# RaduAlexandru/permuto_sdf

Measured on AMD Instinct MI355X. Metric: ray-samples/sec (encode+MLP+composite), higher is better.
Workload: dtype f32 (MLP products on 2 fp16 operand pieces per fp32 value, fp32 accumulation; the 3-piece / 24-bit figure is value_fp32_equivalent_24bit)

## Files before the change

permuto_sdf_amd/csrc/encode.hip:

```cpp
#include <cstdlib>
#include <cstdio>
#include "encode_device.h"
#include <vector>
#include <mutex>
#include <cstring>

namespace {

template <int P, int F, bool PLAIN = false>
__global__ void __launch_bounds__(PSDF_BLOCK)
    encode_fwd_kernel(int64_t N, int L, uint32_t capacity, EncConv conv, const float* __restrict__ positions,
                      const float* __restrict__ lattice, const float* __restrict__ scale_factor,
                      const float* __restrict__ shifts, const float* __restrict__ window, float points_scaling,
                      int pad_points, const unsigned char* __restrict__ skip, float* __restrict__ sliced,
                      unsigned char* __restrict__ touched, int touch_shift, int blocks_per_level) {
  const int level = blockIdx.y;
  const int64_t ntiles = (N + PSDF_BLOCK - 1) / PSDF_BLOCK;
  for (int64_t tile = blockIdx.x; tile < ntiles; tile += gridDim.x) {
  const int64_t n = tile * PSDF_BLOCK + threadIdx.x;
  if (n >= N) continue;
  if (!PLAIN && skip && skip[n]) continue;
  float pos[P];
  load_pos<P>(positions, n, pos);
  if (level >= L) {
// ... 83 lines not shown
  constexpr int ROW_SHR = 0x110, ROW_SHL = 0x100;
  const int k = (int)key;
  const int kprev = __builtin_amdgcn_update_dpp(0, k, ROW_SHR | 1, 0xf, 0xf, true);
  const float joined = (kprev == k) ? 1.0f : 0.0f;
  float j = joined;
#define PSDF_SCAN_STEP(D)                                                                                        \
  {                                                                                                              \
    _Pragma("unroll") for (int i = 0; i < F; i++) v[i] = __builtin_fmaf(                                         \
        __int_as_float(__builtin_amdgcn_update_dpp(0, __float_as_int(v[i]), ROW_SHR | D, 0xf, 0xf, true)), j, v[i]); \
    j = j * __int_as_float(__builtin_amdgcn_update_dpp(0, __float_as_int(j), ROW_SHR | D, 0xf, 0xf, true));      \
  }
  PSDF_SCAN_STEP(1)
  PSDF_SCAN_STEP(2)
  PSDF_SCAN_STEP(4)
  PSDF_SCAN_STEP(8)
#undef PSDF_SCAN_STEP
  const int next_joined = __builtin_amdgcn_update_dpp(0, __float_as_int(joined), ROW_SHL | 1, 0xf, 0xf, true);
  return key != Q_NONE && next_joined == 0;
}

template <int F, int TOTAL = 8192>
struct ScatterCache {
  static constexpr int SC_SLOTS = TOTAL / F;
  uint32_t* tags;
  float* sums;
  int* stats;
  __device__ __forceinline__ void init(float* lds) {
    tags = reinterpret_cast<uint32_t*>(lds);
    sums = lds + SC_SLOTS;
    stats = reinterpret_cast<int*>(lds + SC_SLOTS + SC_SLOTS * F);
    for (int i = threadIdx.x; i < SC_SLOTS; i += blockDim.x) tags[i] = SC_EMPTY;
    for (int i = threadIdx.x; i < SC_SLOTS * F; i += blockDim.x) sums[i] = 0.f;
    if (threadIdx.x == 0) {
      stats[0] = 0;
      stats[1] = 0;
      stats[2] = 1;
    }
    __syncthreads();
  }
  __device__ __forceinline__ int add(uint32_t row, const float* v, int& hot) {
    const uint32_t slot = (row ^ (row >> 12)) & (SC_SLOTS - 1);
    uint32_t old = tags[slot];
    if (old == SC_EMPTY) old = atomicCAS(&tags[slot], SC_EMPTY, row);
    if (old == SC_EMPTY || old == row) {
      static_assert(F % 2 == 0, "pairs");
#pragma unroll
      for (int f = 0; f < F; f += 2) lds_add_pair(&sums[slot * F + f], v[f], v[f + 1], hot);
      return old == row ? 2 : 1;
    }
    return 0;
  }
  __device__ __forceinline__ void flush(float* __restrict__ table_grad) {
    __syncthreads();
    for (int i = threadIdx.x; i < SC_SLOTS; i += blockDim.x) {
      const uint32_t row = tags[i];
      if (row != SC_EMPTY) {
#pragma unroll
        for (int f = 0; f < F; f++) {
          const float v = sums[i * F + f];
          if (v != 0.f) atomicAdd(table_grad + (int64_t)row * F + f, v);
        }
      }
    }
  }
  static constexpr size_t bytes() { return (size_t)(SC_SLOTS + SC_SLOTS * F + 4) * 4; }
};

template <typename SC>
__device__ __forceinline__ bool cache_vote(SC& sc, int hits, int tries) {
  hits = (int)psdf::wave_sum((float)hits);
  tries = (int)psdf::wave_sum((float)tries);
  if (psdf::lane_id() == 0) {
    atomicAdd(&sc.stats[0], hits);
    atomicAdd(&sc.stats[1], tries);
  }
  __syncthreads();
  return sc.stats[0] * 8 >= sc.stats[1];
}

struct Queues {
  uint16_t* rows;
  float* vals;
  int* tails;
  int cap, np, shift;
};
constexpr int Q_MAX_PARTS = 64;
constexpr int Q_LDS_INTS = 4 * Q_MAX_PARTS + 4;

struct LevelQueues {
  char* rows;
  char* vals;
  uint32_t mask;
};
template <int F>
__device__ __forceinline__ LevelQueues level_queues(const Queues& Q, int level) {
  const int64_t e = (int64_t)level * Q.np * Q.cap;
  return LevelQueues{reinterpret_cast<char*>(Q.rows + e), reinterpret_cast<char*>(Q.vals + e * F), (1u << Q.shift) - 1u};
}
template <int F>
__device__ __forceinline__ void queue_store(const LevelQueues& LQ, uint32_t o, uint32_t row, const float* v) {
  *reinterpret_cast<uint16_t*>(LQ.rows + (o * 2u)) = (uint16_t)(row & LQ.mask);
  if (F == 2) {
    *reinterpret_cast<float2*>(LQ.vals + (o * 8u)) = make_float2(v[0], v[F - 1]);
  } else {
#pragma unroll
    for (int f = 0; f < F; f++) *reinterpret_cast<float*>(LQ.vals + (o * (uint32_t)(F * 4) + (uint32_t)(f * 4))) = v[f];
  }
}

template <int NC, int F>
__device__ __forceinline__ void queue_push(const Queues& Q, int level, int* q_cnt, int* q_base,
                                           const uint32_t (&crow)[NC], const float (&cval)[NC][F],
                                           float* __restrict__ table_grad) {
  int* q_aux = q_base + Q_MAX_PARTS;
  const LevelQueues LQ = level_queues<F>(Q, level);
  if (threadIdx.x < Q.np) q_cnt[threadIdx.x] = 0;
  __syncthreads();
  int slot[NC];
#pragma unroll
  for (int r = 0; r < NC; r++)
    if (crow[r] != Q_NONE) slot[r] = atomicAdd(&q_cnt[crow[r] >> Q.shift], 1);
  __syncthreads();
  if (threadIdx.x < Q.np) {
    const int c = q_cnt[threadIdx.x];
    const int base = c ? atomicAdd(&Q.tails[level * Q.np + threadIdx.x], c) : 0;
    q_base[threadIdx.x] = base;
    q_aux[threadIdx.x] = (int)threadIdx.x * Q.cap + base;
  }
  __syncthreads();
#pragma unroll
  for (int r = 0; r < NC; r++) {
    if (crow[r] == Q_NONE) continue;
    const int part = crow[r] >> Q.shift;
    const int idx = q_base[part] + slot[r];
    if (idx < Q.cap) {
      queue_store<F>(LQ, (uint32_t)(q_aux[part] + slot[r]), crow[r], cval[r]);
    } else {
#pragma unroll
      for (int f = 0; f < F; f++) atomicAdd(table_grad + (int64_t)crow[r] * F + f, cval[r][f]);
    }
  }
}

template <int NC>
__device__ __forceinline__ void queue_push_staged(const Queues& Q, int level, int* q_cnt, int* q_base, int* q_off, int* q_gd,
                                                  float* stage, const uint32_t (&crow)[NC],
                                                  const float (&cval)[NC][2], float* __restrict__ table_grad) {
  uint32_t* st_row = reinterpret_cast<uint32_t*>(stage);
  float2* st_val = reinterpret_cast<float2*>(stage + NC * PSDF_BLOCK);
  const LevelQueues LQ = level_queues<2>(Q, level);
  if (threadIdx.x < Q.np) q_cnt[threadIdx.x] = 0;
  __syncthreads();
  int slot[NC];
#pragma unroll
  for (int r = 0; r < NC; r++)
    if (crow[r] != Q_NONE) slot[r] = atomicAdd(&q_cnt[crow[r] >> Q.shift], 1);
  __syncthreads();
  if (threadIdx.x < 64) {
    const int lane = threadIdx.x;
    const int c = lane < Q.np ? q_cnt[lane] : 0;
    const int incl = psdf::wave_incl_scan_add_i(c);
    if (lane < Q.np) {
      const int base = c ? atomicAdd(&Q.tails[level * Q.np + lane], c) : 0;
      const int off = incl - c;
      q_off[lane] = off;
      q_base[lane] = base - off;
      q_gd[lane] = lane * Q.cap + base - off;
      if (lane == Q.np - 1) q_off[Q.np] = incl;
// ... 348 lines not shown
#pragma unroll
  for (int li = 0; li < POS_LPB; li++) {
    const int level = blockIdx.y * POS_LPB + li;
    if (level >= Lt) break;
    float g[F];
#pragma unroll
    for (int f = 0; f < F; f++)
      g[f] = (level < L || (level - L) * F + f < P || pad_points) ? grad_sliced[((int64_t)level * F + f) * N + n] : 0.f;
    if (level >= L) {
      const int e = level - L;
#pragma unroll
      for (int f = 0; f < F; f++) {
        const int d = e * F + f;
#pragma unroll
        for (int i = 0; i < P; i++)
          if (i == d) gp[i] = gp[i] + g[f] * points_scaling;
      }
      continue;
    }
    float sfl[P], shl[P];
#pragma unroll
    for (int i = 0; i < P; i++) {
      sfl[i] = scale_factor[level * P + i];
      shl[i] = shifts[level * P + i];
    }
    const float w = window[level];
    if (w == 0.f) continue;
    const int64_t tbase = (int64_t)level * capacity * F;
    Simplex<P> s;
    compute_simplex<P>(pos, shl, sfl, s, conv.tie_later);
    float dbary[P + 2];
#pragma unroll
    for (int k = 0; k <= P + 1; k++) dbary[k] = 0.f;
    uint32_t rows[P + 1];
    vertex_rows<P>(s, capacity, rows, conv.hash_c);
#pragma unroll
    for (int r = 0; r <= P; r++) {
      const uint32_t row = rows[r];
#pragma unroll
      for (int f = 0; f < F; f++) dbary[r] = dbary[r] + lattice[tbase + (int64_t)row * F + f] * w * g[f];
    }
    dbary[P + 1] = dbary[P + 1] + dbary[0];
    float dE[P + 1];
    const float invp = 1.0f / (P + 1);
#pragma unroll
    for (int i = 0; i <= P; i++) {
      float a = 0.f, b = 0.f;
#pragma unroll
      for (int k = 0; k <= P + 1; k++) {
        if (k == P - s.rank[i]) a = dbary[k];
        if (k == P + 1 - s.rank[i]) b = dbary[k];
      }
      dE[i] = (a - b) * invp;
    }
#pragma unroll
    for (int i = 0; i < P; i++) {
      float acc = 0.f;
#pragma unroll
      for (int j = 0; j <= i; j++) acc = acc + dE[j];
      acc = acc - dE[i + 1] * (float)(i + 1);
      gp[i] = gp[i] + acc * sfl[i];
    }
  }
  if (PARTIAL) {
#pragma unroll
    for (int i = 0; i < P; i++) grad_positions[((int64_t)blockIdx.y * N + n) * P + i] = gp[i];
  } else {
#pragma unroll
    for (int i = 0; i < P; i++) atomicAdd(grad_positions + n * P + i, gp[i]);
  }
}

__global__ void __launch_bounds__(PSDF_BLOCK)
    encode_bwd_pos_reduce_kernel(int64_t NP, int P, int groups, const float* __restrict__ partial,
                                 const unsigned char* __restrict__ skip, float* __restrict__ grad_positions) {
  const int64_t e = (int64_t)blockIdx.x * PSDF_BLOCK + threadIdx.x;
  if (e >= NP) return;
  if (skip && skip[e / P]) return;
  float s = partial[e];
  for (int g = 1; g < groups; g++) s = s + partial[(int64_t)g * NP + e];
  grad_positions[e] = grad_positions[e] + s;
}

template <int F>
__global__ void __launch_bounds__(1024)
    encode_bwd_reduce_kernel(uint32_t capacity, Queues Q, float* __restrict__ grad_lattice) {
  extern __shared__ __align__(16) float tab[];
  const int part = blockIdx.x, level = blockIdx.y;
  int n = Q.tails[level * Q.np + part];
  if (n == 0) return;
  if (n > Q.cap) n = Q.cap;
  const int rpp = 1 << Q.shift;
  for (int i = threadIdx.x; i < rpp * F; i += blockDim.x) tab[i] = 0.f;
  __syncthreads();
  const int64_t qb = ((int64_t)level * Q.np + part) * Q.cap;
  const uint16_t* __restrict__ rows = Q.rows + qb;
  const float* __restrict__ vals = Q.vals + qb * F;
#if !defined(PSDF_ENC_REDUCE_U)
#define PSDF_ENC_REDUCE_U 8
#endif
  constexpr int U = PSDF_ENC_REDUCE_U;
  int hot = 0;
  for (int base = 0; base < n; base += U * (int)blockDim.x) {
    int row[U];
    float v[U][F];
#pragma unroll
    for (int u = 0; u < U; u++) {
      const int i = base + u * (int)blockDim.x + (int)threadIdx.x;
      row[u] = (i < n) ? (int)rows[i] : -1;
      if (F == 2) {
        const float2 t = (i < n) ? *reinterpret_cast<const float2*>(vals + (int64_t)i * 2) : make_float2(0.f, 0.f);
        v[u][0] = t.x;
        v[u][F - 1] = t.y;
      } else {
#pragma unroll
        for (int f = 0; f < F; f++) v[u][f] = (i < n) ? vals[(int64_t)i * F + f] : 0.f;
      }
    }
#pragma unroll
    for (int u = 0; u < U; u++)
      if (row[u] >= 0) {
#pragma unroll
        for (int f = 0; f < F; f += 2) lds_add_pair(&tab[row[u] * F + f], v[u][f], v[u][f + 1], hot);
      }
  }
  __syncthreads();
  const int64_t row0 = (int64_t)part << Q.shift;
  int64_t nrows = (int64_t)capacity - row0;
  if (nrows > rpp) nrows = rpp;
  float* __restrict__ out = grad_lattice + ((int64_t)level * capacity + row0) * F;
  for (int64_t i = threadIdx.x; i < nrows * F; i += blockDim.x) {
    const float v = tab[i];
    if (v != 0.f) out[i] = out[i] + v;
  }
}

template <int P, int F, bool LATTICE>
__global__ void __launch_bounds__(PSDF_BLOCK)
    encode_dbl_bwd_kernel(int64_t N, int L, uint32_t capacity, EncConv conv, const float* __restrict__ positions,
                          const float* __restrict__ lattice, const float* __restrict__ scale_factor,
                          const float* __restrict__ shifts, const float* __restrict__ window, float points_scaling,
                          int pad_points, const float* __restrict__ dd_positions, const float* __restrict__ grad_sliced,
                          float* __restrict__ grad_lattice, float* __restrict__ grad_grad_sliced) {
  extern __shared__ __align__(16) float lds[];
  const int level = blockIdx.y;
  const int64_t ntiles = (N + PSDF_BLOCK - 1) / PSDF_BLOCK;
  if (level >= L) {
    const int e = level - L;
    for (int64_t tile = blockIdx.x; tile < ntiles; tile += gridDim.x) {
      const int64_t n = tile * PSDF_BLOCK + threadIdx.x;
      if (n >= N) continue;
      float u[P];
      load_pos<P>(dd_positions, n, u);
#pragma unroll
      for (int f = 0; f < F; f++) {
        const int d = e * F + f;
        float v = 0.f;
#pragma unroll
        for (int i = 0; i < P; i++)
          if (i == d) v = u[i] * points_scaling;
        if (d < P || pad_points) grad_grad_sliced[((int64_t)level * F + f) * N + n] = v;
      }
    }
    return;
  }
  const float w = window[level];
  if (w == 0.f) {
    for (int64_t tile = blockIdx.x; tile < ntiles; tile += gridDim.x) {
      const int64_t n = tile * PSDF_BLOCK + threadIdx.x;
      if (n >= N) continue;
#pragma unroll
      for (int f = 0; f < F; f++) grad_grad_sliced[((int64_t)level * F + f) * N + n] = 0.f;
    }
    return;
  }
  ScatterCache<F> sc;
  if (LATTICE) sc.init(lds);
  bool use_cache = LATTICE;
  int hot = 0;
  int hits = 0, tries = 0, iter = 0;
  const int64_t tbase = (int64_t)level * capacity * F;
  float sfl[P], shl[P];
#pragma unroll
  for (int i = 0; i < P; i++) {
    sfl[i] = scale_factor[level * P + i];
    shl[i] = shifts[level * P + i];
  }
  for (int64_t tile = blockIdx.x; tile < ntiles; tile += gridDim.x, iter++) {
    const int64_t n = tile * PSDF_BLOCK + threadIdx.x;
    if (n < N) {
      float u[P], pos[P];
      load_pos<P>(dd_positions, n, u);
      load_pos<P>(positions, n, pos);
      Simplex<P> s;
      compute_simplex<P>(pos, shl, sfl, s, conv.tie_later);
      float aE[P + 1];
#pragma unroll
      for (int j = 0; j <= P; j++) aE[j] = 0.f;
#pragma unroll
      for (int k = 0; k < P; k++) {
        const float us = u[k] * sfl[k];
#pragma unroll
        for (int j = 0; j <= k; j++) aE[j] = aE[j] + us;
        aE[k + 1] = aE[k + 1] - us * (float)(k + 1);
      }
      float q[P + 2];
#pragma unroll
      for (int k = 0; k <= P + 1; k++) q[k] = 0.f;
      const float invp = 1.0f / (P + 1);
#pragma unroll
      for (int i = 0; i <= P; i++) {
        const float t = aE[i] * invp;
#pragma unroll
        for (int k = 0; k <= P + 1; k++) {
          if (k == P - s.rank[i]) q[k] = q[k] + t;
          if (k == P + 1 - s.rank[i]) q[k] = q[k] - t;
// ... 86 lines not shown
                                  pad, grad_sliced, skip, grad_positions, st, true);
  else if (N >= ((int64_t)1 << 17))
    launch_bwd_pos_lpb<P_, F_, 2>(N, nr_levels, Lt, capacity, positions, lattice, scale_factor, shifts, window, points_scaling,
                                  pad, grad_sliced, skip, grad_positions, st, false);
  else
    launch_bwd_pos_lpb<P_, F_, 8>(N, nr_levels, Lt, capacity, positions, lattice, scale_factor, shifts, window, points_scaling,
                                  pad, grad_sliced, skip, grad_positions, st, false);
}

extern "C" {

int64_t psdf_encode_convention(int which) {
  switch (which) {
    case 0: return (int64_t)psdf::enc_conv_state().hash_c;
    case 1: return (int64_t)psdf::enc_conv_state().tie_later;
    case 2: return PSDF_ENC_SCALE_SQRT_TERM;
    case 3: return PSDF_ENC_SCALE_INV_STDDEV;
    case 4: return PSDF_ENC_CONCAT_DEFAULT_LAYOUT;
    default: return -1;
  }
}

int psdf_encode_set_conventions(uint32_t hash_multiplier, int rank_tie_raises_later) {
  if (hash_multiplier == 0u || (rank_tie_raises_later != 0 && rank_tie_raises_later != 1)) return PSDF_ERR_ARG;
  psdf::enc_conv_state() = EncConv{hash_multiplier, (uint32_t)rank_tie_raises_later};
  return PSDF_OK;
}

static int device_cus();
static int encode_forward_impl(int pos_dim, int nr_feat, int64_t N, int nr_levels, int capacity, const float* positions,
                               const float* lattice, const float* scale_factor, const float* shifts, const float* window,
                               int concat_points, float points_scaling, const unsigned char* skip, float* sliced,
                               void* stream, unsigned char* touched = nullptr, int touch_shift = 0) {
  if (N == 0) return PSDF_OK;
  if (N < 0 || nr_levels <= 0 || capacity <= 0 || !positions || !lattice || !sliced || !concat_ok(concat_points))
    return PSDF_ERR_ARG;
  if ((int64_t)capacity * nr_feat * 4 > 0xffffffffll) return PSDF_ERR_UNSUPPORTED;
  hipStream_t st = (hipStream_t)stream;
  const int Lt = nr_levels + extra_levels(pos_dim, nr_feat, concat_points);
  dim3 grid(psdf_blocks(N, PSDF_BLOCK), Lt);
  static const int fwd_env = getenv("PSDF_ENC_FWD_WGS") ? atoi(getenv("PSDF_ENC_FWD_WGS")) : -1;
  const int fwd_wgs = fwd_env >= 0 ? fwd_env : device_cus() * 8;
  if (fwd_wgs > 0 && (int)grid.x > fwd_wgs) grid.x = fwd_wgs;
#define FWD_(P_, F_, PL_)                                                                                      \
  hipLaunchKernelGGL((encode_fwd_kernel<P_, F_, PL_>), grid, dim3(PSDF_BLOCK), 0, st, N, nr_levels, (uint32_t)capacity, psdf::enc_conv_state(), \
                     positions, lattice, scale_factor, shifts, window, points_scaling, pad_points(concat_points), skip, sliced,  \
                     touched, touch_shift, (capacity + (1 << touch_shift) - 1) >> touch_shift)
#define FWD(P_, F_)                          \
  do {                                       \
    if (!skip && !touched) FWD_(P_, F_, true); \
    else FWD_(P_, F_, false);                \
  } while (0)
  if (pos_dim == 3 && nr_feat == 2)
    FWD(3, 2);
  else if (pos_dim == 4 && nr_feat == 2)
    FWD(4, 2);
  else if (pos_dim == 2 && nr_feat == 2)
    FWD(2, 2);
  else if (pos_dim == 3 && nr_feat == 4)
    FWD(3, 4);
  else
    return PSDF_ERR_UNSUPPORTED;
#undef FWD
#undef FWD_
  PSDF_LAUNCH_CHECK();
  return PSDF_OK;
}

int psdf_encode_forward(int pos_dim, int nr_feat, int64_t N, int nr_levels, int capacity, const float* positions,
                        const float* lattice, const float* scale_factor, const float* shifts, const float* window,
                        int concat_points, float points_scaling, float* sliced, void* stream) {
  return encode_forward_impl(pos_dim, nr_feat, N, nr_levels, capacity, positions, lattice, scale_factor, shifts, window,
                             concat_points, points_scaling, nullptr, sliced, stream);
}

int psdf_encode_forward_masked(int pos_dim, int nr_feat, int64_t N, int nr_levels, int capacity, const float* positions,
                               const float* lattice, const float* scale_factor, const float* shifts, const float* window,
                               int concat_points, float points_scaling, const unsigned char* skip, float* sliced,
                               void* stream) {
  return encode_forward_impl(pos_dim, nr_feat, N, nr_levels, capacity, positions, lattice, scale_factor, shifts, window,
                             concat_points, points_scaling, skip, sliced, stream);
}

static bool queue_plan(int pos_dim, int nr_feat, int64_t N, int nr_levels, int capacity, Queues& Q, int64_t& bytes) {
  bytes = 0;
  static const int64_t min_n = getenv("PSDF_ENC_QUEUE_MIN_N") ? atoll(getenv("PSDF_ENC_QUEUE_MIN_N")) : ((int64_t)1 << 13);
  if (N < min_n) return false;
  const int base = (nr_feat <= 2) ? 14 : (nr_feat <= 4 ? 13 : 12);
  static const int delta = getenv("PSDF_ENC_QUEUE_SLICE_LOG2_DELTA") ? atoi(getenv("PSDF_ENC_QUEUE_SLICE_LOG2_DELTA")) : 1;
  int shift = base - (delta < 0 ? 0 : (delta > 3 ? 3 : delta));
  while (shift < base && ((capacity + (1 << shift) - 1) >> shift) > Q_MAX_PARTS) shift++;
  const int rpp = 1 << shift;
  const int np = (capacity + rpp - 1) / rpp;
  if (np > Q_MAX_PARTS || rpp * nr_feat * 4 > 128 * 1024) return false;
  const int64_t contrib = (int64_t)(pos_dim + 1) * N;
  const int64_t cap = (contrib / np) + (contrib / np) / 4 + 4096;
  if (cap > 0x7fffffff) return false;
  if ((int64_t)np * cap * (nr_feat * 4 > 2 ? nr_feat * 4 : 2) > 0xffffffffll) return false;
  Q.cap = (int)cap;
  Q.np = np;
  Q.shift = shift;
  const int64_t entries = (int64_t)nr_levels * np * cap;
  const int64_t rows_b = (entries * 2 + 255) & ~(int64_t)255, vals_b = (entries * nr_feat * 4 + 255) & ~(int64_t)255;
  bytes = rows_b + vals_b + (((int64_t)nr_levels * np * 4 + 255) & ~(int64_t)255) + 1024;
  return true;
}
static void queue_carve(void* ws, int nr_feat, int nr_levels, Queues& Q) {
  const int64_t entries = (int64_t)nr_levels * Q.np * Q.cap;
  const int64_t rows_b = (entries * 2 + 255) & ~(int64_t)255, vals_b = (entries * nr_feat * 4 + 255) & ~(int64_t)255;
  char* p = (char*)ws;
  Q.rows = (uint16_t*)p;
  Q.vals = (float*)(p + rows_b);
  Q.tails = (int*)(p + rows_b + vals_b);
}

int psdf_encode_forward_mark(int pos_dim, int nr_feat, int64_t N, int nr_levels, int capacity, const float* positions,
                             const float* lattice, const float* scale_factor, const float* shifts, const float* window,
                             int concat_points, float points_scaling, float* sliced, unsigned char* touched_blocks,
                             int block_rows_log2, void* stream) {
  if (!touched_blocks || block_rows_log2 < 0 || block_rows_log2 > 20) return PSDF_ERR_ARG;
  return encode_forward_impl(pos_dim, nr_feat, N, nr_levels, capacity, positions, lattice, scale_factor, shifts, window,
                             concat_points, points_scaling, nullptr, sliced, stream, touched_blocks, block_rows_log2);
}

int64_t psdf_encode_backward_workspace_bytes(int pos_dim, int nr_feat, int64_t N, int nr_levels, int capacity) {
  Queues Q{};
  int64_t bytes = 0;
  queue_plan(pos_dim, nr_feat, N, nr_levels, capacity, Q, bytes);
  return bytes;
}

static int device_cus() {
  static int cus[64] = {};
  int dev = 0;
  if (hipGetDevice(&dev) != hipSuccess || dev < 0 || dev >= 64) return 256;
  if (cus[dev] == 0) {
    int n = 0;
    if (hipDeviceGetAttribute(&n, hipDeviceAttributeMultiprocessorCount, dev) != hipSuccess || n <= 0) n = 256;
    cus[dev] = n;
  }
  return cus[dev];
}

}

namespace {
struct EncBalance {
  int levels = 0, total = 0, kind = 0, bucket = -1;
  const void* ident = nullptr;
  uint32_t gen = 0;
  uint64_t last_use = 0;
  std::vector<int> counts;
  uint32_t* times[2] = {nullptr, nullptr};
  int device = -1;
};
constexpr int BAL_MAX_WG = 8192, BAL_MIN_PER_LEVEL = 4, BAL_STATES = 16;
std::mutex g_shares_mu;
std::vector<int> g_last_shares;

bool encode_balance(int nr_levels, int64_t N, int total, int64_t super_tiles, LevelPlan& plan, const void* ident, int kind = 0) {
  static const bool off = getenv("PSDF_ENC_BWD_BALANCE") && atoi(getenv("PSDF_ENC_BWD_BALANCE")) == 0;
  static std::mutex mu;
  static EncBalance states[BAL_STATES];
  static uint64_t tick = 0;
  if (off || nr_levels > 40 || total > BAL_MAX_WG || total < nr_levels * BAL_MIN_PER_LEVEL || N < ((int64_t)1 << 18)) return false;
  std::lock_guard<std::mutex> lock(mu);
  int bucket = 0;
  for (int64_t v = N; v > 1; v >>= 1) bucket += 4;
  {
    const int64_t top = (int64_t)1 << (bucket / 4);
    bucket += (int)(((N - top) * 4) / top);
  }
  int device = -1;
  (void)hipGetDevice(&device);
  EncBalance* Bp = nullptr;
  for (auto& st_ : states)
    if (st_.times[0] && st_.ident == ident && st_.device == device && st_.kind == kind && st_.levels == nr_levels && st_.bucket == bucket &&
        st_.total == total)
      Bp = &st_;
  if (!Bp) {
    for (auto& st_ : states)
      if (!Bp || st_.last_use < Bp->last_use) Bp = &st_;
    if (!Bp->times[0]) {
      for (int i = 0; i < 2; i++) {
        void* h = nullptr;
        if (hipHostMalloc(&h, BAL_MAX_WG * sizeof(uint32_t), hipHostMallocMapped) != hipSuccess || !h) {
          (void)hipGetLastError();
          if (i == 1) (void)hipHostFree(Bp->times[0]);
          Bp->times[0] = Bp->times[1] = nullptr;
          return false;
        }
        Bp->times[i] = (uint32_t*)h;
      }
    }
    memset(Bp->times[0], 0, BAL_MAX_WG * sizeof(uint32_t));
    memset(Bp->times[1], 0, BAL_MAX_WG * sizeof(uint32_t));
    Bp->levels = 0;
  }
  EncBalance& B = *Bp;
  B.last_use = ++tick;
  if (!B.times[0] || !B.times[1]) return false;
  const int cap = (int)(super_tiles < total ? super_tiles : total);
  if (B.levels != nr_levels || (int)B.counts.size() != nr_levels) {
    B.levels = nr_levels;
    B.kind = kind;
    B.ident = ident;
    B.device = device;
    B.bucket = bucket;
    B.total = total;
    B.counts.assign(nr_levels, total / nr_levels);
  } else {
    const volatile uint32_t* t = B.times[B.gen & 1];
    std::vector<double> work(nr_levels, 0.0);
    bool complete = true;
    int id = 0;
    double sum = 0.0;
    for (int l = 0; l < nr_levels && complete; l++) {
      double acc = 0.0;
      for (int b = 0; b < B.counts[l]; b++, id++) {
        const uint32_t v = t[id];
        if ((v >> 24) != (B.gen & 255u) || (v & 0xFFFFFFu) == 0u) {
          complete = false;
          break;
        }
        acc += (double)(v & 0xFFFFFFu);
      }
      work[l] = acc;
      sum += acc;
    }
    if (complete && sum > 0.0) {
      std::vector<double> want(nr_levels);
      for (int l = 0; l < nr_levels; l++) want[l] = 0.5 * B.counts[l] + 0.5 * total * work[l] / sum;
      int used = 0;
      for (int l = 0; l < nr_levels; l++) {
        int c = (int)(want[l] + 0.5);
        c = c < BAL_MIN_PER_LEVEL ? BAL_MIN_PER_LEVEL : (c > cap ? cap : c);
        B.counts[l] = c;
        used += c;
      }
      while (used > total) {
        int big = 0;
        for (int l = 1; l < nr_levels; l++)
          if (B.counts[l] > B.counts[big]) big = l;
        if (B.counts[big] <= BAL_MIN_PER_LEVEL) break;
        B.counts[big]--;
        used--;
      }
    }
  }
  B.gen++;
  plan.n = nr_levels;
  plan.gen = B.gen;
  plan.times = B.times[B.gen & 1];
  int at = 0;
  for (int l = 0; l < nr_levels; l++) {
    if (B.counts[l] > cap) B.counts[l] = cap;
    if (B.counts[l] < 1) B.counts[l] = 1;
    plan.first[l] = (uint16_t)at;
    at += B.counts[l];
  }
  plan.first[nr_levels] = (uint16_t)at;
  {
    std::lock_guard<std::mutex> l2(g_shares_mu);
    g_last_shares = B.counts;
  }
  return at <= BAL_MAX_WG;
}
}

extern "C" {

int psdf_encode_backward_level_shares(int* counts, int max_levels) {
  std::lock_guard<std::mutex> lock(g_shares_mu);
  const int n = (int)g_last_shares.size();
  for (int l = 0; l < n && l < max_levels; l++) counts[l] = g_last_shares[l];
  return n;
}

int psdf_encode_backward_ws(int pos_dim, int nr_feat, int64_t N, int nr_levels, int capacity, const float* positions,
                            const float* lattice, const float* scale_factor, const float* shifts, const float* window,
                            int concat_points, float points_scaling, const float* grad_sliced, float* grad_lattice,
                            float* grad_positions, void* workspace, int64_t workspace_bytes, void* stream) {
  if (N == 0 || (!grad_lattice && !grad_positions)) return PSDF_OK;
  if (N < 0 || nr_levels <= 0 || capacity <= 0 || !positions || !lattice || !grad_sliced || !concat_ok(concat_points))
    return PSDF_ERR_ARG;
  hipStream_t st = (hipStream_t)stream;
  const int Lt = nr_levels + ((grad_positions != nullptr) ? extra_levels(pos_dim, nr_feat, concat_points) : 0);
  const unsigned nb = psdf_blocks(N, PSDF_BLOCK);
  static const int wg_cap_env = getenv("PSDF_ENC_BWD_WG_PER_LEVEL") ? atoi(getenv("PSDF_ENC_BWD_WG_PER_LEVEL")) : 0;
  const unsigned wg_cap = wg_cap_env > 0 ? (unsigned)wg_cap_env : 512u;
  dim3 grid(nb < wg_cap ? nb : wg_cap, Lt);
  static const bool pos_fused = getenv("PSDF_ENC_POS_FUSED") && atoi(getenv("PSDF_ENC_POS_FUSED")) != 0;
  Queues Q{};
  int64_t need = 0;
  const bool use_queue = grad_lattice && workspace && queue_plan(pos_dim, nr_feat, N, nr_levels, capacity, Q, need) &&
                         workspace_bytes >= need;
  if (use_queue) {
    grid.x = 128;
    queue_carve(workspace, nr_feat, nr_levels, Q);
#if defined(PSDF_ENC_PROFILE)
    hipError_t e = hipMemsetAsync(Q.tails, 0, (size_t)nr_levels * Q.np * sizeof(int) + 1024, st);
#else
    hipError_t e = hipMemsetAsync(Q.tails, 0, (size_t)nr_levels * Q.np * sizeof(int), st);
#endif
    if (e != hipSuccess) return (int)e;
  }
#define BWD(P_, F_, A_, B_, Q_)                                                                                  \
  hipLaunchKernelGGL((encode_bwd_kernel<P_, F_, A_, B_, Q_>), grid, dim3(PSDF_BLOCK),                             \
                     ((A_) ? ScatterCache<F_, ((Q_) ? 4096 : 8192)>::bytes() + Q_LDS_INTS * sizeof(int) : 0), st, N, \
                     nr_levels,                                                                                    \
                     (uint32_t)capacity, psdf::enc_conv_state(), positions, lattice, scale_factor, shifts, window, points_scaling,        \
                     grad_sliced, grad_lattice, grad_positions, Q)
#define BWD_PLAN(P_, F_)                                                                                          \
  hipLaunchKernelGGL((encode_bwd_kernel<P_, F_, true, false, true>), dim3(plan.first[nr_levels]), dim3(PSDF_BLOCK), \
                     (ScatterCache<F_, 4096>::bytes() + Q_LDS_INTS * sizeof(int)), st, N, nr_levels,    \
                     (uint32_t)capacity, psdf::enc_conv_state(), positions, lattice, scale_factor, shifts, window, \
                     points_scaling, grad_sliced, grad_lattice, (float*)nullptr, Q, (const float*)nullptr,          \
                     (float*)nullptr, 0, (const float*)nullptr, plan)
#define BWD_PF(P_, F_)                                                                                           \
  do {                                                                                                           \
    LevelPlan plan{};                                                                                            \
    bool balanced = false;                                                                                       \
    if (use_queue) {                                                                                             \
      int per_cu = 0;                                                                                            \
      const size_t shm = ScatterCache<F_, 4096>::bytes() + Q_LDS_INTS * sizeof(int);                  \
      const hipError_t eo =                                                                                      \
          (grad_positions && pos_fused) ? hipOccupancyMaxActiveBlocksPerMultiprocessor(                                        \
                               &per_cu, encode_bwd_kernel<P_, F_, true, true, true>, PSDF_BLOCK, shm)            \
                         : hipOccupancyMaxActiveBlocksPerMultiprocessor(                                        \
                               &per_cu, encode_bwd_kernel<P_, F_, true, false, true>, PSDF_BLOCK, shm);          \
      if (eo == hipSuccess && per_cu > 0) {                                                                      \
        int64_t gx = (int64_t)per_cu * device_cus() / nr_levels;                                                 \
        const int64_t super_tiles = (N + (int64_t)PSDF_BLOCK * QUEUE_SPT - 1) / ((int64_t)PSDF_BLOCK * QUEUE_SPT); \
        if (gx > super_tiles) gx = super_tiles;                                                                  \
        grid.x = (unsigned)(gx < 1 ? 1 : gx);                                                                    \
                   \
        if (!(grad_positions && pos_fused))                                                                      \
          balanced = encode_balance(nr_levels, N, per_cu * device_cus(), super_tiles, plan, lattice);                     \
      } else {                                                                                                   \
        (void)hipGetLastError();                                                                                 \
      }                                                                                                          \
    }                                                                                                            \
    if (use_queue && grad_positions && !pos_fused) {                                                             \
       \
       \
         \
      grid.y = nr_levels;                                                                                        \
      if (balanced) BWD_PLAN(P_, F_); else BWD(P_, F_, true, false, true);                                       \
      launch_bwd_pos<P_, F_>(N, nr_levels, Lt, capacity, positions, lattice, scale_factor, shifts, window,        \
                             points_scaling, pad_points(concat_points), grad_sliced, (const unsigned char*)nullptr, \
                             grad_positions, st);                                                                 \
    } else if (use_queue && grad_positions)                                                                      \
      BWD(P_, F_, true, true, true);                                                                             \
    else if (use_queue) {                                                                                        \
      if (balanced) BWD_PLAN(P_, F_); else BWD(P_, F_, true, false, true);                                       \
    }                                                                                                            \
    else if (grad_lattice && grad_positions)                                                                     \
      BWD(P_, F_, true, true, false);                                                                            \
    else if (grad_lattice)                                                                                       \
      BWD(P_, F_, true, false, false);                                                                           \
    else                                                                                                         \
      launch_bwd_pos<P_, F_>(N, nr_levels, Lt, capacity, positions, lattice, scale_factor, shifts, window,        \
                             points_scaling, pad_points(concat_points), grad_sliced, (const unsigned char*)nullptr, \
                             grad_positions, st);                                                                 \
    if (use_queue) {                                                                                             \
      const size_t lds_b = (size_t)(1 << Q.shift) * F_ * sizeof(float);                                          \
      hipError_t e2 = hipFuncSetAttribute((const void*)encode_bwd_reduce_kernel<F_>,                              \
                                          hipFuncAttributeMaxDynamicSharedMemorySize, (int)lds_b);                \
      if (e2 != hipSuccess) return (int)e2;                                                                      \
      hipLaunchKernelGGL((encode_bwd_reduce_kernel<F_>), dim3(Q.np, nr_levels), dim3(1024), lds_b, st,            \
                         (uint32_t)capacity, Q, grad_lattice);                                                   \
    }                                                                                                            \
  } while (0)
  if (pos_dim == 3 && nr_feat == 2)
    BWD_PF(3, 2);
  else if (pos_dim == 4 && nr_feat == 2)
    BWD_PF(4, 2);
  else if (pos_dim == 2 && nr_feat == 2)
    BWD_PF(2, 2);
  else if (pos_dim == 3 && nr_feat == 4)
    BWD_PF(3, 4);
  else
    return PSDF_ERR_UNSUPPORTED;
#undef BWD_PF
#undef BWD_PLAN
#undef BWD
  psdf::g_last_path[psdf::PATH_ENCODE_BWD] = use_queue ? 2 : (grad_lattice ? 1 : 3);
#if defined(PSDF_ENC_PROFILE)
  if (use_queue) {
    static int calls = 0;
    if (++calls == 8) {
      (void)hipStreamSynchronize(st);
      int prof[192];
      (void)hipMemcpy(prof, Q.tails + nr_levels * Q.np, sizeof(prof), hipMemcpyDeviceToHost);
      std::vector<int> tails((size_t)nr_levels * Q.np);
      (void)hipMemcpy(tails.data(), Q.tails, tails.size() * sizeof(int), hipMemcpyDeviceToHost);
      for (int l = 0; l < nr_levels; l++) {
        long long queued = 0;
        for (int q = 0; q < Q.np; q++) queued += tails[(size_t)l * Q.np + q];
        fprintf(stderr, "[enc-profile] level %2d: max %8d ticks, mean %8.0f ticks, cache kept by %d of %u workgroups, queued %lld of %lld "
                "contributions (%.1f %%)\n", l, prof[l], 64.0 * prof[64 + l] / grid.x, prof[128 + l], grid.x, queued,
                (long long)N * (pos_dim + 1), 100.0 * queued / ((double)N * (pos_dim + 1)));
      }
    }
  }
#endif
  PSDF_LAUNCH_CHECK();
  return PSDF_OK;
}

int psdf_encode_backward(int pos_dim, int nr_feat, int64_t N, int nr_levels, int capacity, const float* positions,
                         const float* lattice, const float* scale_factor, const float* shifts, const float* window,
                         int concat_points, float points_scaling, const float* grad_sliced, float* grad_lattice,
                         float* grad_positions, void* stream) {
  return psdf_encode_backward_ws(pos_dim, nr_feat, N, nr_levels, capacity, positions, lattice, scale_factor, shifts,
                                 window, concat_points, points_scaling, grad_sliced, grad_lattice, grad_positions,
                                 nullptr, 0, stream);
}

int psdf_encode_backward_positions_masked(int pos_dim, int nr_feat, int64_t N, int nr_levels, int capacity,
                                          const float* positions, const float* lattice, const float* scale_factor,
                                          const float* shifts, const float* window, int concat_points, float points_scaling,
                                          const float* grad_sliced, const unsigned char* skip, float* grad_positions,
                                          void* stream) {
  if (N == 0) return PSDF_OK;
  if (N < 0 || nr_levels <= 0 || capacity <= 0 || !positions || !lattice || !grad_sliced || !grad_positions ||
      !concat_ok(concat_points))
    return PSDF_ERR_ARG;
  hipStream_t st = (hipStream_t)stream;
  const int Lt = nr_levels + extra_levels(pos_dim, nr_feat, concat_points);
#define POS(P_, F_)                                                                                                  \
  launch_bwd_pos<P_, F_>(N, nr_levels, Lt, capacity, positions, lattice, scale_factor, shifts, window, points_scaling, \
                         pad_points(concat_points), grad_sliced, skip, grad_positions, st)
  if (pos_dim == 3 && nr_feat == 2)
    POS(3, 2);
  else if (pos_dim == 4 && nr_feat == 2)
    POS(4, 2);
  else if (pos_dim == 2 && nr_feat == 2)
    POS(2, 2);
  else if (pos_dim == 3 && nr_feat == 4)
    POS(3, 4);
  else
    return PSDF_ERR_UNSUPPORTED;
#undef POS
  PSDF_LAUNCH_CHECK();
  return PSDF_OK;
}

int psdf_encode_double_backward_ws(int pos_dim, int nr_feat, int64_t N, int nr_levels, int capacity,
                                   const float* positions, const float* lattice, const float* scale_factor,
                                   const float* shifts, const float* window, int concat_points, float points_scaling,
                                   const float* dd_positions, const float* grad_sliced, float* grad_lattice,
                                   float* grad_grad_sliced, const float* grad_sliced_direct, void* workspace,
                                   int64_t workspace_bytes, void* stream) {
  if (N == 0) return PSDF_OK;
  if (N < 0 || nr_levels <= 0 || capacity <= 0 || !positions || !lattice || !dd_positions || !grad_sliced ||
      (!grad_grad_sliced && !grad_lattice) || (grad_sliced_direct && !grad_lattice) || !concat_ok(concat_points))
    return PSDF_ERR_ARG;
  hipStream_t st = (hipStream_t)stream;
  const int Lt = nr_levels + extra_levels(pos_dim, nr_feat, concat_points);
  const unsigned nb = psdf_blocks(N, PSDF_BLOCK);
  {
    Queues Q{};
    int64_t need = 0;
    if (grad_lattice && workspace && queue_plan(pos_dim, nr_feat, N, nr_levels, capacity, Q, need) && workspace_bytes >= need) {
      queue_carve(workspace, nr_feat, nr_levels, Q);
      hipError_t e = hipMemsetAsync(Q.tails, 0, (size_t)nr_levels * Q.np * sizeof(int), st);
      if (e != hipSuccess) return (int)e;
#define DBLQ(P_, F_)                                                                                                     \
  do {                                                                                                                   \
    auto kern = encode_bwd_kernel<P_, F_, true, false, true, true>;                                                      \
    const size_t shm = ScatterCache<F_, 4096>::bytes() + Q_LDS_INTS * sizeof(int);                            \
    int per_cu = 0;                                                                                                      \
    int64_t gx = 128;                                                                                                    \
    if (hipOccupancyMaxActiveBlocksPerMultiprocessor(&per_cu, kern, PSDF_BLOCK, shm) == hipSuccess && per_cu > 0)        \
      gx = (int64_t)per_cu * device_cus() / nr_levels;            \
    else                                                                                                                 \
      (void)hipGetLastError();                                                                                           \
    const int64_t super_tiles = (N + (int64_t)PSDF_BLOCK * QUEUE_SPT - 1) / ((int64_t)PSDF_BLOCK * QUEUE_SPT);           \
    if (gx > super_tiles) gx = super_tiles;                                                                              \
     \
                       \
    LevelPlan plan{};                                                                                                    \
    dim3 g2((unsigned)(gx < 1 ? 1 : gx), Lt);                                                                            \
    if (per_cu > 0 && encode_balance(Lt, N, per_cu * device_cus(), super_tiles, plan, lattice, 1)) g2 = dim3(plan.first[Lt]);       \
    else plan = LevelPlan{};                                                                                             \
    hipLaunchKernelGGL(kern, g2, dim3(PSDF_BLOCK), shm, st, N, nr_levels,                                                \
                       (uint32_t)capacity, psdf::enc_conv_state(), positions, lattice, scale_factor, shifts, window,     \
                       points_scaling, grad_sliced, grad_lattice, (float*)nullptr, Q, dd_positions, grad_grad_sliced,    \
                       pad_points(concat_points), grad_sliced_direct, plan);                                             \
    const size_t lds_b = (size_t)(1 << Q.shift) * F_ * sizeof(float);                                                    \
    hipError_t e2 = hipFuncSetAttribute((const void*)encode_bwd_reduce_kernel<F_>,                                       \
                                        hipFuncAttributeMaxDynamicSharedMemorySize, (int)lds_b);                         \
    if (e2 != hipSuccess) return (int)e2;                                                                                \
    hipLaunchKernelGGL((encode_bwd_reduce_kernel<F_>), dim3(Q.np, nr_levels), dim3(1024), lds_b, st, (uint32_t)capacity, \
                       Q, grad_lattice);                                                                                 \
  } while (0)
      if (pos_dim == 3 && nr_feat == 2)
        DBLQ(3, 2);
      else if (pos_dim == 4 && nr_feat == 2)
        DBLQ(4, 2);
      else if (pos_dim == 2 && nr_feat == 2)
        DBLQ(2, 2);
      else if (pos_dim == 3 && nr_feat == 4)
        DBLQ(3, 4);
      else
        return PSDF_ERR_UNSUPPORTED;
#undef DBLQ
      PSDF_LAUNCH_CHECK();
      return PSDF_OK;
    }
  }
  if (grad_sliced_direct) {
    const int rc = psdf_encode_backward_ws(pos_dim, nr_feat, N, nr_levels, capacity, positions, lattice, scale_factor, shifts,
                                           window, concat_points, points_scaling, grad_sliced_direct, grad_lattice, nullptr,
                                           nullptr, 0, stream);
    if (rc != PSDF_OK) return rc;
  }
  if (!grad_grad_sliced) {
    grad_grad_sliced = (float*)psdf::stream_scratch((size_t)Lt * nr_feat * N * sizeof(float), st);
    if (!grad_grad_sliced) return PSDF_ERR_UNSUPPORTED;
  }
  static const int wg_cap_env = getenv("PSDF_ENC_BWD_WG_PER_LEVEL") ? atoi(getenv("PSDF_ENC_BWD_WG_PER_LEVEL")) : 0;
  const unsigned wg_cap = wg_cap_env > 0 ? (unsigned)wg_cap_env : 512u;
  dim3 grid(nb < wg_cap ? nb : wg_cap, Lt);
#define DBL(P_, F_)                                                                                              \
  do {                                                                                                           \
    if (grad_lattice)                                                                                            \
      hipLaunchKernelGGL((encode_dbl_bwd_kernel<P_, F_, true>), grid, dim3(PSDF_BLOCK), ScatterCache<F_>::bytes(), \
                         st, N, nr_levels, (uint32_t)capacity, psdf::enc_conv_state(), positions, lattice, scale_factor, shifts, window,   \
                         points_scaling, pad_points(concat_points), dd_positions, grad_sliced, grad_lattice,       \
                         grad_grad_sliced);                                                                        \
    else                                                                                                         \
      hipLaunchKernelGGL((encode_dbl_bwd_kernel<P_, F_, false>), grid, dim3(PSDF_BLOCK), 0, st, N, nr_levels,      \
                         (uint32_t)capacity, psdf::enc_conv_state(), positions, lattice, scale_factor, shifts, window, points_scaling,     \
                         pad_points(concat_points), dd_positions, grad_sliced, grad_lattice, grad_grad_sliced);    \
  } while (0)
  if (pos_dim == 3 && nr_feat == 2)
    DBL(3, 2);
  else if (pos_dim == 4 && nr_feat == 2)
    DBL(4, 2);
  else if (pos_dim == 2 && nr_feat == 2)
    DBL(2, 2);
  else if (pos_dim == 3 && nr_feat == 4)
    DBL(3, 4);
  else
    return PSDF_ERR_UNSUPPORTED;
#undef DBL
  PSDF_LAUNCH_CHECK();
  return PSDF_OK;
}

int psdf_encode_double_backward(int pos_dim, int nr_feat, int64_t N, int nr_levels, int capacity,
                                const float* positions, const float* lattice, const float* scale_factor,
                                const float* shifts, const float* window, int concat_points, float points_scaling,
                                const float* dd_positions, const float* grad_sliced, float* grad_lattice,
                                float* grad_grad_sliced, void* stream) {
  return psdf_encode_double_backward_ws(pos_dim, nr_feat, N, nr_levels, capacity, positions, lattice, scale_factor, shifts,
                                        window, concat_points, points_scaling, dd_positions, grad_sliced, grad_lattice,
                                        grad_grad_sliced, nullptr, nullptr, 0, stream);
}

}
```

Baseline: 982.8 million.

## Load-balance queue reduce across persistent workgroups with split-queue slab combining

Replaces the one-workgroup-per-(level,partition) queue reduce with a persistent grid that prefix-sums the queue lengths and gives each workgroup an equal slice of total work. Queues split across workgroups write partial LDS images to global slabs, and a ticket counter picks the last finisher to combine them into the lattice gradient. The aligned interior now loads rows and values in groups of 8 entries. This targets load imbalance from uneven queue sizes, at the cost of extra slab traffic, atomics, a larger workspace, and an LDS-capacity check that can disable the queue path.

```diff
diff --git a/permuto_sdf_amd/csrc/encode.hip b/permuto_sdf_amd/csrc/encode.hip
--- a/permuto_sdf_amd/csrc/encode.hip
+++ b/permuto_sdf_amd/csrc/encode.hip
@@ -189,8 +189,11 @@
   uint16_t* rows;
   float* vals;
   int* tails;
+  int* tickets;
+  float* slabs;
   int cap, np, shift;
 };
+constexpr int R_MAX_WG = 512;
 constexpr int Q_MAX_PARTS = 64;
 constexpr int Q_LDS_INTS = 4 * Q_MAX_PARTS + 4;
 
@@ -705,56 +708,192 @@
   grad_positions[e] = grad_positions[e] + s;
 }
 
+__device__ __forceinline__ long long reduce_cut(const long long* pre, int nq, long long P, int w) {
+  const long long x = (long long)w * P;
+  if (x >= pre[nq]) return pre[nq];
+  int lo = 0, hi = nq - 1;
+  while (lo < hi) {
+    const int mid = (lo + hi + 1) >> 1;
+    if (pre[mid] <= x) lo = mid; else hi = mid - 1;
+  }
+  return (pre[lo + 1] - pre[lo] < P) ? pre[lo] : x;
+}
+
+__device__ __forceinline__ const float* reduce_slab(const float* slabs, long long p, long long p_first, int nimg) {
+  return slabs + (int64_t)(2 * p + (p == p_first ? 1 : 0)) * nimg;
+}
+__device__ __forceinline__ void reduce_write(float* __restrict__ out, const float* a, int cnt, const float* slabs,
+                                             long long p_first, long long p_last, long long self, int nimg) {
+  if ((((uintptr_t)out) & 15) == 0 && (cnt & 3) == 0) {
+    for (int i = threadIdx.x * 4; i < cnt; i += blockDim.x * 4) {
+      float4 v = *reinterpret_cast<const float4*>(a + i);
+      for (long long p = p_first; p <= p_last; p++) {
+        if (p == self) continue;
+        const float4 t = *reinterpret_cast<const float4*>(reduce_slab(slabs, p, p_first, nimg) + i);
+        v.x += t.x; v.y += t.y; v.z += t.z; v.w += t.w;
+      }
+      if (v.x != 0.f || v.y != 0.f || v.z != 0.f || v.w != 0.f) {
+        float4* o = reinterpret_cast<float4*>(out + i);
+        float4 r = *o;
+        r.x += v.x; r.y += v.y; r.z += v.z; r.w += v.w;
+        *o = r;
+      }
+    }
+  } else {
+    for (int i = threadIdx.x; i < cnt; i += blockDim.x) {
+      float v = a[i];
+      for (long long p = p_first; p <= p_last; p++)
+        if (p != self) v += reduce_slab(slabs, p, p_first, nimg)[i];
+      if (v != 0.f) out[i] = out[i] + v;
+    }
+  }
+}
+
 template <int F>
 __global__ void __launch_bounds__(1024)
-    encode_bwd_reduce_kernel(uint32_t capacity, Queues Q, float* __restrict__ grad_lattice) {
+    encode_bwd_reduce_kernel(uint32_t capacity, Queues Q, float* __restrict__ grad_lattice, int nq) {
   extern __shared__ __align__(16) float tab[];
-  const int part = blockIdx.x, level = blockIdx.y;
-  int n = Q.tails[level * Q.np + part];
-  if (n == 0) return;
-  if (n > Q.cap) n = Q.cap;
   const int rpp = 1 << Q.shift;
-  for (int i = threadIdx.x; i < rpp * F; i += blockDim.x) tab[i] = 0.f;
+  const int nimg = rpp * F;
+  long long* pre = reinterpret_cast<long long*>(tab + nimg);
+  __shared__ int s_last;
+  const int w = blockIdx.x;
+  if (threadIdx.x < 64) {
+    const int lane = threadIdx.x, per = (nq + 63) / 64, q0 = lane * per;
+    long long run = 0;
+    for (int q = q0; q < q0 + per && q < nq; q++) {
+      int n = Q.tails[q];
+      n = n > Q.cap ? Q.cap : n;
+      run += n > 0 ? (long long)n + rpp : 0;
+    }
+    long long incl = run;
+#pragma unroll
+    for (int d = 1; d < 64; d <<= 1) {
+      const long long t = __shfl_up(incl, d, 64);
+      if (lane >= d) incl += t;
+    }
+    long long x = incl - run;
+    for (int q = q0; q < q0 + per && q < nq; q++) {
+      pre[q] = x;
+      int n = Q.tails[q];
+      n = n > Q.cap ? Q.cap : n;
+      x += n > 0 ? (long long)n + rpp : 0;
+    }
+    if (lane == 63) pre[nq] = incl;
+  }
   __syncthreads();
-  const int64_t qb = ((int64_t)level * Q.np + part) * Q.cap;
-  const uint16_t* __restrict__ rows = Q.rows + qb;
-  const float* __restrict__ vals = Q.vals + qb * F;
+  if (pre[nq] == 0) return;
+  const long long P = (pre[nq] + gridDim.x - 1) / gridDim.x;
+  const long long a = reduce_cut(pre, nq, P, w), b = reduce_cut(pre, nq, P, w + 1);
+  if (a >= b) return;
+  int q = 0;
+  {
+    int lo = 0, hi = nq - 1;
+    while (lo < hi) {
+      const int mid = (lo + hi + 1) >> 1;
+      if (pre[mid] <= a) lo = mid; else hi = mid - 1;
+    }
+    q = lo;
+  }
 #if !defined(PSDF_ENC_REDUCE_U)
 #define PSDF_ENC_REDUCE_U 8
 #endif
   constexpr int U = PSDF_ENC_REDUCE_U;
+  static_assert(U % 8 == 0, "groups of 8 entries");
+  constexpr int NG = U / 8;
   int hot = 0;
-  for (int base = 0; base < n; base += U * (int)blockDim.x) {
-    int row[U];
-    float v[U][F];
-#pragma unroll
-    for (int u = 0; u < U; u++) {
-      const int i = base + u * (int)blockDim.x + (int)threadIdx.x;
-      row[u] = (i < n) ? (int)rows[i] : -1;
-      if (F == 2) {
-        const float2 t = (i < n) ? *reinterpret_cast<const float2*>(vals + (int64_t)i * 2) : make_float2(0.f, 0.f);
-        v[u][0] = t.x;
-        v[u][F - 1] = t.y;
-      } else {
-#pragma unroll
-        for (int f = 0; f < F; f++) v[u][f] = (i < n) ? vals[(int64_t)i * F + f] : 0.f;
-      }
-    }
-#pragma unroll
-    for (int u = 0; u < U; u++)
-      if (row[u] >= 0) {
-#pragma unroll
-        for (int f = 0; f < F; f += 2) lds_add_pair(&tab[row[u] * F + f], v[u][f], v[u][f + 1], hot);
-      }
-  }
-  __syncthreads();
-  const int64_t row0 = (int64_t)part << Q.shift;
-  int64_t nrows = (int64_t)capacity - row0;
-  if (nrows > rpp) nrows = rpp;
-  float* __restrict__ out = grad_lattice + ((int64_t)level * capacity + row0) * F;
-  for (int64_t i = threadIdx.x; i < nrows * F; i += blockDim.x) {
-    const float v = tab[i];
-    if (v != 0.f) out[i] = out[i] + v;
+  for (; q < nq && pre[q] < b; q++) {
+    int n = Q.tails[q];
+    n = n > Q.cap ? Q.cap : n;
+    if (n <= 0) continue;
+    const long long e0 = pre[q] + rpp;
+    long long lo = a - e0, hi = b - e0;
+    lo = lo < 0 ? 0 : (lo > n ? n : lo);
+    hi = hi < 0 ? 0 : (hi > n ? n : hi);
+    if (lo >= hi) continue;
+    const int level = q / Q.np, part = q - level * Q.np;
+    for (int i = threadIdx.x * 4; i < nimg; i += blockDim.x * 4) *reinterpret_cast<float4*>(tab + i) = make_float4(0.f, 0.f, 0.f, 0.f);
+    __syncthreads();
+    const int64_t qb = (int64_t)q * Q.cap;
+    const uint16_t* __restrict__ rows = Q.rows + qb;
+    const float* __restrict__ vals = Q.vals + qb * F;
+    const int ilo = (int)lo, ihi = (int)hi;
+    const int alo = (ilo + 7) & ~7;
+    const int ahi = ihi & ~7;
+    {
+      const int t = threadIdx.x;
+      int i = -1;
+      if (alo >= ahi) {
+        if (t < ihi - ilo) i = ilo + t;
+      } else if (t < alo - ilo) {
+        i = ilo + t;
+      } else if (t >= 8 && t - 8 < ihi - ahi) {
+        i = ahi + (t - 8);
+      }
+      if (i >= 0) {
+        float v[F];
+#pragma unroll
+        for (int f = 0; f < F; f++) v[f] = vals[(int64_t)i * F + f];
+        const int r = rows[i];
+#pragma unroll
+        for (int f = 0; f < F; f += 2) lds_add_pair(&tab[r * F + f], v[f], v[f + 1], hot);
+      }
+    }
+    if (alo < ahi) {
+      const int g0 = alo >> 3, ng = (ahi - alo) >> 3;
+      const uint4* __restrict__ rg = reinterpret_cast<const uint4*>(rows) + g0;
+      const float4* __restrict__ vg = reinterpret_cast<const float4*>(vals) + (int64_t)g0 * (2 * F);
+      for (int base = 0; base < ng; base += NG * (int)blockDim.x) {
+        uint4 rr[NG];
+        float4 vv[NG][2 * F];
+#pragma unroll
+        for (int u = 0; u < NG; u++) {
+          const int g = base + u * (int)blockDim.x + (int)threadIdx.x;
+          if (g < ng) {
+            rr[u] = rg[g];
+#pragma unroll
+            for (int k = 0; k < 2 * F; k++) vv[u][k] = vg[(int64_t)g * (2 * F) + k];
+          }
+        }
+#pragma unroll
+        for (int u = 0; u < NG; u++) {
+          const int g = base + u * (int)blockDim.x + (int)threadIdx.x;
+          if (g < ng) {
+            const uint32_t rw[4] = {rr[u].x, rr[u].y, rr[u].z, rr[u].w};
+            const float* fv = reinterpret_cast<const float*>(&vv[u][0]);
+#pragma unroll
+            for (int e = 0; e < 8; e++) {
+              const int r = (int)((rw[e >> 1] >> ((e & 1) * 16)) & 0xffffu);
+#pragma unroll
+              for (int f = 0; f < F; f += 2) lds_add_pair(&tab[r * F + f], fv[e * F + f], fv[e * F + f + 1], hot);
+            }
+          }
+        }
+      }
+    }
+    __syncthreads();
+    const int64_t row0 = (int64_t)part << Q.shift;
+    int64_t nrows = (int64_t)capacity - row0;
+    if (nrows > rpp) nrows = rpp;
+    float* __restrict__ out = grad_lattice + ((int64_t)level * capacity + row0) * F;
+    const int cnt = (int)(nrows * F);
+    const long long p_first = e0 / P, p_last = (pre[q + 1] - 1) / P;
+    if (pre[q + 1] - pre[q] < P || p_first == p_last) {
+      reduce_write(out, tab, cnt, Q.slabs, 1, 0, -1, nimg);
+    } else {
+      float* mine = const_cast<float*>(reduce_slab(Q.slabs, w, p_first, nimg));
+      for (int i = threadIdx.x * 4; i < cnt; i += blockDim.x * 4)
+        *reinterpret_cast<float4*>(mine + i) = *reinterpret_cast<const float4*>(tab + i);
+      __threadfence();
+      __syncthreads();
+      if (threadIdx.x == 0) s_last = atomicAdd(&Q.tickets[q], 1) == (int)(p_last - p_first);
+      __syncthreads();
+      if (s_last) {
+        __threadfence();
+        reduce_write(out, tab, cnt, Q.slabs, p_first, p_last, w, nimg);
+      }
+    }
+    __syncthreads();
   }
 }
 
@@ -1007,6 +1146,7 @@
                              concat_points, points_scaling, skip, sliced, stream);
 }
 
+static int64_t queue_counter_bytes(int nq) { return (((int64_t)2 * nq + 256) * 4 + 255) & ~(int64_t)255; }
 static bool queue_plan(int pos_dim, int nr_feat, int64_t N, int nr_levels, int capacity, Queues& Q, int64_t& bytes) {
   bytes = 0;
   static const int64_t min_n = getenv("PSDF_ENC_QUEUE_MIN_N") ? atoll(getenv("PSDF_ENC_QUEUE_MIN_N")) : ((int64_t)1 << 13);
@@ -1018,8 +1158,9 @@
   const int rpp = 1 << shift;
   const int np = (capacity + rpp - 1) / rpp;
   if (np > Q_MAX_PARTS || rpp * nr_feat * 4 > 128 * 1024) return false;
+  if ((int64_t)rpp * nr_feat * 4 + ((int64_t)nr_levels * np + 1) * 8 > 160 * 1024) return false;
   const int64_t contrib = (int64_t)(pos_dim + 1) * N;
-  const int64_t cap = (contrib / np) + (contrib / np) / 4 + 4096;
+  const int64_t cap = ((contrib / np) + (contrib / np) / 4 + 4096 + 7) & ~(int64_t)7;
   if (cap > 0x7fffffff) return false;
   if ((int64_t)np * cap * (nr_feat * 4 > 2 ? nr_feat * 4 : 2) > 0xffffffffll) return false;
   Q.cap = (int)cap;
@@ -1027,7 +1168,7 @@
   Q.shift = shift;
   const int64_t entries = (int64_t)nr_levels * np * cap;
   const int64_t rows_b = (entries * 2 + 255) & ~(int64_t)255, vals_b = (entries * nr_feat * 4 + 255) & ~(int64_t)255;
-  bytes = rows_b + vals_b + (((int64_t)nr_levels * np * 4 + 255) & ~(int64_t)255) + 1024;
+  bytes = rows_b + vals_b + queue_counter_bytes(nr_levels * np) + (int64_t)2 * R_MAX_WG * rpp * nr_feat * 4;
   return true;
 }
 static void queue_carve(void* ws, int nr_feat, int nr_levels, Queues& Q) {
@@ -1037,6 +1178,8 @@
   Q.rows = (uint16_t*)p;
   Q.vals = (float*)(p + rows_b);
   Q.tails = (int*)(p + rows_b + vals_b);
+  Q.tickets = Q.tails + nr_levels * Q.np + 256;
+  Q.slabs = (float*)(p + rows_b + vals_b + queue_counter_bytes(nr_levels * Q.np));
 }
 
 int psdf_encode_forward_mark(int pos_dim, int nr_feat, int64_t N, int nr_levels, int capacity, const float* positions,
@@ -1191,6 +1334,24 @@
   }
   return at <= BAL_MAX_WG;
 }
+
+size_t reduce_lds_bytes(int nr_feat, int nq, int shift) { return ((size_t)nr_feat << shift) * sizeof(float) + ((size_t)nq + 1) * 8; }
+template <int F>
+int launch_reduce(int capacity, int nr_levels, const Queues& Q, float* grad_lattice, hipStream_t st) {
+  const int nq = nr_levels * Q.np;
+  const size_t lds_b = reduce_lds_bytes(F, nq, Q.shift);
+  hipError_t e = hipFuncSetAttribute((const void*)encode_bwd_reduce_kernel<F>, hipFuncAttributeMaxDynamicSharedMemorySize, (int)lds_b);
+  if (e != hipSuccess) return (int)e;
+  int per_cu = 0;
+  if (hipOccupancyMaxActiveBlocksPerMultiprocessor(&per_cu, encode_bwd_reduce_kernel<F>, 1024, lds_b) != hipSuccess || per_cu < 1) {
+    (void)hipGetLastError();
+    per_cu = 1;
+  }
+  int G = per_cu * device_cus();
+  if (G > R_MAX_WG) G = R_MAX_WG;
+  hipLaunchKernelGGL((encode_bwd_reduce_kernel<F>), dim3(G), dim3(1024), lds_b, st, (uint32_t)capacity, Q, grad_lattice, nq);
+  return (int)hipSuccess;
+}
 }
 
 extern "C" {
@@ -1223,11 +1384,7 @@
   if (use_queue) {
     grid.x = 128;
     queue_carve(workspace, nr_feat, nr_levels, Q);
-#if defined(PSDF_ENC_PROFILE)
-    hipError_t e = hipMemsetAsync(Q.tails, 0, (size_t)nr_levels * Q.np * sizeof(int) + 1024, st);
-#else
-    hipError_t e = hipMemsetAsync(Q.tails, 0, (size_t)nr_levels * Q.np * sizeof(int), st);
-#endif
+    hipError_t e = hipMemsetAsync(Q.tails, 0, (size_t)queue_counter_bytes(nr_levels * Q.np), st);
     if (e != hipSuccess) return (int)e;
   }
 #define BWD(P_, F_, A_, B_, Q_)                                                                                  \
@@ -1289,12 +1446,8 @@
                              points_scaling, pad_points(concat_points), grad_sliced, (const unsigned char*)nullptr, \
                              grad_positions, st);                                                                 \
     if (use_queue) {                                                                                             \
-      const size_t lds_b = (size_t)(1 << Q.shift) * F_ * sizeof(float);                                          \
-      hipError_t e2 = hipFuncSetAttribute((const void*)encode_bwd_reduce_kernel<F_>,                              \
-                                          hipFuncAttributeMaxDynamicSharedMemorySize, (int)lds_b);                \
-      if (e2 != hipSuccess) return (int)e2;                                                                      \
-      hipLaunchKernelGGL((encode_bwd_reduce_kernel<F_>), dim3(Q.np, nr_levels), dim3(1024), lds_b, st,            \
-                         (uint32_t)capacity, Q, grad_lattice);                                                   \
+      const int e2 = launch_reduce<F_>(capacity, nr_levels, Q, grad_lattice, st);                               \
+      if (e2 != hipSuccess) return e2;                                                                           \
     }                                                                                                            \
   } while (0)
   if (pos_dim == 3 && nr_feat == 2)
@@ -1390,7 +1543,7 @@
     int64_t need = 0;
     if (grad_lattice && workspace && queue_plan(pos_dim, nr_feat, N, nr_levels, capacity, Q, need) && workspace_bytes >= need) {
       queue_carve(workspace, nr_feat, nr_levels, Q);
-      hipError_t e = hipMemsetAsync(Q.tails, 0, (size_t)nr_levels * Q.np * sizeof(int), st);
+      hipError_t e = hipMemsetAsync(Q.tails, 0, (size_t)queue_counter_bytes(nr_levels * Q.np), st);
       if (e != hipSuccess) return (int)e;
 #define DBLQ(P_, F_)                                                                                                     \
   do {                                                                                                                   \
@@ -1414,12 +1567,8 @@
                        (uint32_t)capacity, psdf::enc_conv_state(), positions, lattice, scale_factor, shifts, window,     \
                        points_scaling, grad_sliced, grad_lattice, (float*)nullptr, Q, dd_positions, grad_grad_sliced,    \
                        pad_points(concat_points), grad_sliced_direct, plan);                                             \
-    const size_t lds_b = (size_t)(1 << Q.shift) * F_ * sizeof(float);                                                    \
-    hipError_t e2 = hipFuncSetAttribute((const void*)encode_bwd_reduce_kernel<F_>,                                       \
-                                        hipFuncAttributeMaxDynamicSharedMemorySize, (int)lds_b);                         \
-    if (e2 != hipSuccess) return (int)e2;                                                                                \
-    hipLaunchKernelGGL((encode_bwd_reduce_kernel<F_>), dim3(Q.np, nr_levels), dim3(1024), lds_b, st, (uint32_t)capacity, \
-                       Q, grad_lattice);                                                                                 \
+    const int e2 = launch_reduce<F_>(capacity, nr_levels, Q, grad_lattice, st);                                        \
+    if (e2 != hipSuccess) return e2;                                                                                     \
   } while (0)
       if (pos_dim == 3 && nr_feat == 2)
         DBLQ(3, 2);
```

Result: slower. 731.7 million, median of 2 (-25.5%).
